# zhanxinrui/HDN

Measured on AMD Instinct MI355X. Metric: frames/sec on 127/255 template/search pairs, higher is better.
Workload: dtype f32; 1 GPU; BASELINE configs[1]: batch=64 synthetic 127/255 pairs per GPU, 256-ch features; HIP kernels only: 1x xcorr 31x31(x)61x61 + 6x xcorr 5x5(x)29x29 + 6x circular xcorr 13x13(x)13x13 + 3x PreShareFeature 127x127 + fused DLT/warp + the 2 L1 scores (one launch); pairs_per_gpu=64, channels=256

## Files before the change

hdn_amd/csrc/share_feature.hip:

```cpp
#include <cstdlib>

#include "hdn_common.h"

#define HDN_ABL_SHARE_FEATURE_0(...) __VA_ARGS__
#define HDN_ABL_SHARE_FEATURE_1(...) __VA_ARGS__
#define HDN_ABL_SHARE_FEATURE_2(...) __VA_ARGS__
#ifdef HDN_ABLATION
#include "ablation/share_feature.inc"
#endif

namespace hdn {

constexpr int SF_ROWS = 4;
constexpr int SF_COLS = 128;

constexpr int SF_W1 = 0, SF_W2 = 36, SF_W3 = 324, SF_ALPHA = 396, SF_BETA = 409;

constexpr int SF_IN_H = SF_ROWS + 6, SF_IN_W = SF_COLS + 6;
constexpr int SF_A_H = SF_ROWS + 4, SF_A_W = SF_COLS + 4;
constexpr int SF_B_H = SF_ROWS + 2, SF_B_W = SF_COLS + 2;
constexpr int SF_IN_N = SF_IN_H * SF_IN_W;
constexpr int SF_A_N = SF_A_H * SF_A_W;
constexpr int SF_B_N = SF_B_H * SF_B_W;
constexpr int SF_LDS_FLOATS = SF_IN_N + 4 * SF_A_N + 8 * SF_B_N;

__global__ __launch_bounds__(HDN_BLOCK) void share_feature_kernel(const float* __restrict__ img,
                                                                  const float* __restrict__ prm,
                                                                  float* __restrict__ out, int H, int W) {
  __shared__ float smem[SF_LDS_FLOATS];
  float* s_in = smem;
  float* s_a = smem + SF_IN_N;
  float* s_b = s_a + 4 * SF_A_N;

  const int tid = threadIdx.x;
  const int c0 = blockIdx.x * SF_COLS;
  const int r0 = blockIdx.y * SF_ROWS;
  const size_t plane = size_t(blockIdx.z) * H * W;
  const float* __restrict__ src = img + plane;

  for (int idx = tid; idx < SF_IN_N; idx += HDN_BLOCK) {
    const int r = idx / SF_IN_W, c = idx - r * SF_IN_W;
    const int gr = r0 - 3 + r, gc = c0 - 3 + c;
    float v = 0.f;
    if (gr >= 0 && gr < H && gc >= 0 && gc < W) v = src[gr * W + gc];
    s_in[idx] = v;
  }
  __syncthreads();

  for (int idx = tid; idx < SF_A_N; idx += HDN_BLOCK) {
    const int r = idx / SF_A_W, c = idx - r * SF_A_W;
    const int gr = r0 - 2 + r, gc = c0 - 2 + c;
    float acc[4] = {0.f, 0.f, 0.f, 0.f};
#pragma unroll
    for (int ky = 0; ky < 3; ++ky)
#pragma unroll
      for (int kx = 0; kx < 3; ++kx) {
        const float v = s_in[(r + ky) * SF_IN_W + c + kx];
#pragma unroll
        for (int co = 0; co < 4; ++co) acc[co] = __builtin_fmaf(v, prm[SF_W1 + (ky * 3 + kx) * 4 + co], acc[co]);
      }
    const bool inside = gr >= 0 && gr < H && gc >= 0 && gc < W;
#pragma unroll
    for (int co = 0; co < 4; ++co) {
      const float y = __builtin_fmaf(acc[co], prm[SF_ALPHA + co], prm[SF_BETA + co]);
      s_a[co * SF_A_N + idx] = inside ? fmaxf(y, 0.f) : 0.f;
    }
  }
  __syncthreads();

  for (int idx = tid; idx < SF_B_N; idx += HDN_BLOCK) {
    const int r = idx / SF_B_W, c = idx - r * SF_B_W;
    const int gr = r0 - 1 + r, gc = c0 - 1 + c;
    float acc[8];
#pragma unroll
    for (int co = 0; co < 8; ++co) acc[co] = 0.f;
#pragma unroll
    for (int ci = 0; ci < 4; ++ci)
#pragma unroll
      for (int ky = 0; ky < 3; ++ky)
#pragma unroll
        for (int kx = 0; kx < 3; ++kx) {
          const float v = s_a[ci * SF_A_N + (r + ky) * SF_A_W + c + kx];
#pragma unroll
          for (int co = 0; co < 8; ++co)
            acc[co] = __builtin_fmaf(v, prm[SF_W2 + (((ci >> 1) * 9 + ky * 3 + kx) * 8 + co) * 2 + (ci & 1)], acc[co]);
        }
    const bool inside = gr >= 0 && gr < H && gc >= 0 && gc < W;
#pragma unroll
    for (int co = 0; co < 8; ++co) {
      const float y = __builtin_fmaf(acc[co], prm[SF_ALPHA + 4 + co], prm[SF_BETA + 4 + co]);
      s_b[co * SF_B_N + idx] = inside ? fmaxf(y, 0.f) : 0.f;
    }
  }
  __syncthreads();

  for (int idx = tid; idx < SF_ROWS * SF_COLS; idx += HDN_BLOCK) {
    const int r = idx / SF_COLS, c = idx - r * SF_COLS;
    const int gr = r0 + r, gc = c0 + c;
    if (gr >= H || gc >= W) continue;
    float acc = 0.f;
#pragma unroll
    for (int ci = 0; ci < 8; ++ci)
#pragma unroll
      for (int ky = 0; ky < 3; ++ky)
#pragma unroll
        for (int kx = 0; kx < 3; ++kx)
          acc = __builtin_fmaf(s_b[ci * SF_B_N + (r + ky) * SF_B_W + c + kx],
                               prm[SF_W3 + ((ci >> 1) * 9 + ky * 3 + kx) * 2 + (ci & 1)], acc);
    const float y = __builtin_fmaf(acc, prm[SF_ALPHA + 12], prm[SF_BETA + 12]);
    out[plane + size_t(gr) * W + gc] = fmaxf(y, 0.f);
  }
}

namespace sfv {
typedef const float __attribute__((address_space(4))) cfloat;
typedef float f16v __attribute__((ext_vector_type(16)));
typedef float f8v __attribute__((ext_vector_type(8)));
typedef float f4v_ __attribute__((ext_vector_type(4)));
typedef const f16v __attribute__((address_space(4), aligned(4))) c16;
typedef const f8v __attribute__((address_space(4), aligned(4))) c8;
typedef const f4v_ __attribute__((address_space(4), aligned(4))) c4;
typedef const float2v __attribute__((address_space(4), aligned(4))) c2;

__device__ __forceinline__ const cfloat* opaque(const float* p) {
  uint64_t a = reinterpret_cast<uint64_t>(p);
  asm volatile("" : "+s"(a));
  return (const cfloat*)a;
}
__device__ __forceinline__ float from_prev_lane(float v) {
  return __builtin_bit_cast(float, __builtin_amdgcn_update_dpp(0, __builtin_bit_cast(int, v), 0x138, 0xf, 0xf, true));
}
__device__ __forceinline__ float from_next_lane(float v) {
  return __builtin_bit_cast(float, __builtin_amdgcn_update_dpp(0, __builtin_bit_cast(int, v), 0x130, 0xf, 0xf, true));
}

#define SFV_FMA_LO(a, v, w) "v_pk_fma_f32 " a ", " v ", " w ", " a " op_sel_hi:[1,0,1]\n\t"
#define SFV_FMA_HI(a, v, w) "v_pk_fma_f32 " a ", " v ", " w ", " a " op_sel:[0,1,0] op_sel_hi:[1,1,1]\n\t"
#define SFV_MUL_LO(a, v, w) "v_pk_mul_f32 " a ", " v ", " w " op_sel_hi:[1,0]\n\t"
#define SFV_MUL_HI(a, v, w) "v_pk_mul_f32 " a ", " v ", " w " op_sel:[0,1] op_sel_hi:[1,1]\n\t"
#define SFV_PAIR(w, k) __builtin_shufflevector(w, w, 2 * (k), 2 * (k) + 1)

template <bool INIT>
__device__ __forceinline__ void tap16(float2v (&acc)[8], float2v ve, float2v vo, const cfloat* wp) {
  const f16v w = *reinterpret_cast<const c16*>(wp);
  if constexpr (INIT) {
    asm(SFV_MUL_LO("%0", "%8", "%10") SFV_MUL_LO("%1", "%8", "%11") SFV_MUL_LO("%2", "%8", "%12") SFV_MUL_LO("%3", "%8", "%13")
        SFV_MUL_LO("%4", "%8", "%14") SFV_MUL_LO("%5", "%8", "%15") SFV_MUL_LO("%6", "%8", "%16") SFV_MUL_LO("%7", "%8", "%17")
        SFV_FMA_HI("%0", "%9", "%10") SFV_FMA_HI("%1", "%9", "%11") SFV_FMA_HI("%2", "%9", "%12") SFV_FMA_HI("%3", "%9", "%13")
        SFV_FMA_HI("%4", "%9", "%14") SFV_FMA_HI("%5", "%9", "%15") SFV_FMA_HI("%6", "%9", "%16") SFV_FMA_HI("%7", "%9", "%17")
        : "=&v"(acc[0]), "=&v"(acc[1]), "=&v"(acc[2]), "=&v"(acc[3]), "=&v"(acc[4]), "=&v"(acc[5]), "=&v"(acc[6]), "=&v"(acc[7])
        : "v"(ve), "v"(vo), "s"(SFV_PAIR(w, 0)), "s"(SFV_PAIR(w, 1)), "s"(SFV_PAIR(w, 2)), "s"(SFV_PAIR(w, 3)), "s"(SFV_PAIR(w, 4)),
          "s"(SFV_PAIR(w, 5)), "s"(SFV_PAIR(w, 6)), "s"(SFV_PAIR(w, 7)));
  } else {
    asm(SFV_FMA_LO("%0", "%8", "%10") SFV_FMA_LO("%1", "%8", "%11") SFV_FMA_LO("%2", "%8", "%12") SFV_FMA_LO("%3", "%8", "%13")
        SFV_FMA_LO("%4", "%8", "%14") SFV_FMA_LO("%5", "%8", "%15") SFV_FMA_LO("%6", "%8", "%16") SFV_FMA_LO("%7", "%8", "%17")
        SFV_FMA_HI("%0", "%9", "%10") SFV_FMA_HI("%1", "%9", "%11") SFV_FMA_HI("%2", "%9", "%12") SFV_FMA_HI("%3", "%9", "%13")
        SFV_FMA_HI("%4", "%9", "%14") SFV_FMA_HI("%5", "%9", "%15") SFV_FMA_HI("%6", "%9", "%16") SFV_FMA_HI("%7", "%9", "%17")
        : "+v"(acc[0]), "+v"(acc[1]), "+v"(acc[2]), "+v"(acc[3]), "+v"(acc[4]), "+v"(acc[5]), "+v"(acc[6]), "+v"(acc[7])
        : "v"(ve), "v"(vo), "s"(SFV_PAIR(w, 0)), "s"(SFV_PAIR(w, 1)), "s"(SFV_PAIR(w, 2)), "s"(SFV_PAIR(w, 3)), "s"(SFV_PAIR(w, 4)),
          "s"(SFV_PAIR(w, 5)), "s"(SFV_PAIR(w, 6)), "s"(SFV_PAIR(w, 7)));
  }
}

template <bool INIT>
__device__ __forceinline__ void scatter18(float2v& o0, float2v& o1, float2v& o2, float2v& o3, float2v& o4, float2v& o5, float2v& o6,
                                          float2v& o7, float2v& o8, float2v be, float2v bo, const cfloat* wp) {
  const f16v w = *reinterpret_cast<const c16*>(wp);
  const float2v w8 = *reinterpret_cast<const c2*>(wp + 16);
  if constexpr (INIT) {
    asm(SFV_MUL_LO("%0", "%9", "%11") SFV_MUL_LO("%1", "%9", "%12") SFV_MUL_LO("%2", "%9", "%13") SFV_FMA_LO("%3", "%9", "%14")
        SFV_FMA_LO("%4", "%9", "%15") SFV_FMA_LO("%5", "%9", "%16") SFV_FMA_LO("%6", "%9", "%17") SFV_FMA_LO("%7", "%9", "%18")
        SFV_FMA_LO("%8", "%9", "%19")
        SFV_FMA_HI("%0", "%10", "%11") SFV_FMA_HI("%1", "%10", "%12") SFV_FMA_HI("%2", "%10", "%13") SFV_FMA_HI("%3", "%10", "%14")
        SFV_FMA_HI("%4", "%10", "%15") SFV_FMA_HI("%5", "%10", "%16") SFV_FMA_HI("%6", "%10", "%17") SFV_FMA_HI("%7", "%10", "%18")
        SFV_FMA_HI("%8", "%10", "%19")
        : "=&v"(o0), "=&v"(o1), "=&v"(o2), "+v"(o3), "+v"(o4), "+v"(o5), "+v"(o6), "+v"(o7), "+v"(o8)
        : "v"(be), "v"(bo), "s"(SFV_PAIR(w, 0)), "s"(SFV_PAIR(w, 1)), "s"(SFV_PAIR(w, 2)), "s"(SFV_PAIR(w, 3)), "s"(SFV_PAIR(w, 4)),
          "s"(SFV_PAIR(w, 5)), "s"(SFV_PAIR(w, 6)), "s"(SFV_PAIR(w, 7)), "s"(w8));
  } else {
    asm(SFV_FMA_LO("%0", "%9", "%11") SFV_FMA_LO("%1", "%9", "%12") SFV_FMA_LO("%2", "%9", "%13") SFV_FMA_LO("%3", "%9", "%14")
        SFV_FMA_LO("%4", "%9", "%15") SFV_FMA_LO("%5", "%9", "%16") SFV_FMA_LO("%6", "%9", "%17") SFV_FMA_LO("%7", "%9", "%18")
        SFV_FMA_LO("%8", "%9", "%19")
        SFV_FMA_HI("%0", "%10", "%11") SFV_FMA_HI("%1", "%10", "%12") SFV_FMA_HI("%2", "%10", "%13") SFV_FMA_HI("%3", "%10", "%14")
        SFV_FMA_HI("%4", "%10", "%15") SFV_FMA_HI("%5", "%10", "%16") SFV_FMA_HI("%6", "%10", "%17") SFV_FMA_HI("%7", "%10", "%18")
        SFV_FMA_HI("%8", "%10", "%19")
        : "+v"(o0), "+v"(o1), "+v"(o2), "+v"(o3), "+v"(o4), "+v"(o5), "+v"(o6), "+v"(o7), "+v"(o8)
        : "v"(be), "v"(bo), "s"(SFV_PAIR(w, 0)), "s"(SFV_PAIR(w, 1)), "s"(SFV_PAIR(w, 2)), "s"(SFV_PAIR(w, 3)), "s"(SFV_PAIR(w, 4)),
          "s"(SFV_PAIR(w, 5)), "s"(SFV_PAIR(w, 6)), "s"(SFV_PAIR(w, 7)), "s"(w8));
  }
}

template <bool INIT>
__device__ __forceinline__ void l1row(float2v (&acc)[4], float2v i0, float2v i1, float2v i2, const cfloat* wp) {
  const f8v w = *reinterpret_cast<const c8*>(wp);
  const f4v_ u = *reinterpret_cast<const c4*>(wp + 8);
  if constexpr (INIT) {
    asm(SFV_MUL_LO("%0", "%4", "%7") SFV_MUL_HI("%1", "%4", "%7") SFV_MUL_LO("%2", "%4", "%8") SFV_MUL_HI("%3", "%4", "%8")
        SFV_FMA_LO("%0", "%5", "%9") SFV_FMA_HI("%1", "%5", "%9") SFV_FMA_LO("%2", "%5", "%10") SFV_FMA_HI("%3", "%5", "%10")
        SFV_FMA_LO("%0", "%6", "%11") SFV_FMA_HI("%1", "%6", "%11") SFV_FMA_LO("%2", "%6", "%12") SFV_FMA_HI("%3", "%6", "%12")
        : "=&v"(acc[0]), "=&v"(acc[1]), "=&v"(acc[2]), "=&v"(acc[3])
        : "v"(i0), "v"(i1), "v"(i2), "s"(SFV_PAIR(w, 0)), "s"(SFV_PAIR(w, 1)), "s"(SFV_PAIR(w, 2)), "s"(SFV_PAIR(w, 3)),
          "s"(SFV_PAIR(u, 0)), "s"(SFV_PAIR(u, 1)));
  } else {
    asm(SFV_FMA_LO("%0", "%4", "%7") SFV_FMA_HI("%1", "%4", "%7") SFV_FMA_LO("%2", "%4", "%8") SFV_FMA_HI("%3", "%4", "%8")
        SFV_FMA_LO("%0", "%5", "%9") SFV_FMA_HI("%1", "%5", "%9") SFV_FMA_LO("%2", "%5", "%10") SFV_FMA_HI("%3", "%5", "%10")
        SFV_FMA_LO("%0", "%6", "%11") SFV_FMA_HI("%1", "%6", "%11") SFV_FMA_LO("%2", "%6", "%12") SFV_FMA_HI("%3", "%6", "%12")
        : "+v"(acc[0]), "+v"(acc[1]), "+v"(acc[2]), "+v"(acc[3])
        : "v"(i0), "v"(i1), "v"(i2), "s"(SFV_PAIR(w, 0)), "s"(SFV_PAIR(w, 1)), "s"(SFV_PAIR(w, 2)), "s"(SFV_PAIR(w, 3)),
          "s"(SFV_PAIR(u, 0)), "s"(SFV_PAIR(u, 1)));
  }
}

__device__ __forceinline__ float2v bn_relu(float2v acc, float2v ab) {
  asm("v_pk_fma_f32 %0, %0, %1, %1 op_sel:[0,0,1] op_sel_hi:[1,0,1]" : "+v"(acc) : "v"(ab));
  float lo = acc.x, hi = acc.y;
  asm("v_max_f32 %0, 0, %0" : "+v"(lo));
  asm("v_max_f32 %0, 0, %0" : "+v"(hi));
  return float2v{lo, hi};
}

struct State {
  float2v in[3][3];
  float2v a[3][4][3];
  float2v o[3][3];
  float2v ab[13];
};

struct Ctx {
  const float* __restrict__ src;
  float* __restrict__ dst;
  const float* __restrict__ prm;
  int H, W, ra, rb;
  int col0, col1;
  bool m0, m1;
};

__device__ __forceinline__ float2v load_row(const Ctx& c, int i) {
  const bool row_ok = i >= 0 && i < c.H;
  const float* __restrict__ p = c.src + (row_ok ? i : 0) * c.W;
  const float x0 = p[c.col0], x1 = p[c.col1];
  return float2v{row_ok && c.m0 ? x0 : 0.f, row_ok && c.m1 ? x1 : 0.f};
}

template <int PH, bool FULL>
__device__ __forceinline__ void step(State& st, const Ctx& c, int i, float2v xin) {
  constexpr int S0 = PH, S1 = (PH + 2) % 3, S2 = (PH + 1) % 3;
  const cfloat* prm = opaque(c.prm);
  st.in[S0][1] = xin;
  st.in[S0][0] = float2v{from_prev_lane(xin.y), xin.x};
  st.in[S0][2] = float2v{xin.y, from_next_lane(xin.x)};

  const int sg = i - 1;
  if (FULL || sg >= c.ra - 2) {
    if (FULL || (sg >= 0 && sg < c.H)) {
      const cfloat* w1 = prm + SF_W1;
      float2v acc[4];
      l1row<true>(acc, st.in[S2][0], st.in[S2][1], st.in[S2][2], w1);
      l1row<false>(acc, st.in[S1][0], st.in[S1][1], st.in[S1][2], w1 + 12);
      l1row<false>(acc, st.in[S0][0], st.in[S0][1], st.in[S0][2], w1 + 24);
#pragma unroll
      for (int co = 0; co < 4; ++co) {
        float2v y = bn_relu(acc[co], st.ab[co]);
        y.x = c.m0 ? y.x : 0.f;
        y.y = c.m1 ? y.y : 0.f;
        st.a[S1][co][1] = y;
        st.a[S1][co][0] = float2v{from_prev_lane(y.y), y.x};
        st.a[S1][co][2] = float2v{y.y, from_next_lane(y.x)};
      }
    } else {
#pragma unroll
      for (int co = 0; co < 4; ++co)
#pragma unroll
        for (int kx = 0; kx < 3; ++kx) st.a[S1][co][kx] = float2v{0.f, 0.f};
    }
  }

  const int rho = i - 2;
  if (FULL || (rho >= c.ra - 1 && rho >= 0 && rho < c.H)) {
    float2v acc[8];
#pragma unroll
    for (int ky = 0; ky < 3; ++ky) {
      constexpr int rs_[3] = {S0, S2, S1};
      const int rs = rs_[ky];
#pragma unroll
      for (int cp = 0; cp < 2; ++cp) {
        const cfloat* w = prm + SF_W2 + (cp * 3 + ky) * 48;
#pragma unroll
        for (int kx = 0; kx < 3; ++kx) {
          if (ky == 0 && cp == 0 && kx == 0) tap16<true>(acc, st.a[rs][2 * cp][kx], st.a[rs][2 * cp + 1][kx], w + kx * 16);
          else tap16<false>(acc, st.a[rs][2 * cp][kx], st.a[rs][2 * cp + 1][kx], w + kx * 16);
        }
      }
    }
#pragma unroll
    for (int co = 0; co < 8; ++co) acc[co] = bn_relu(acc[co], st.ab[4 + co]);
    const cfloat* w3 = prm + SF_W3;
    scatter18<true>(st.o[S1][0], st.o[S1][1], st.o[S1][2], st.o[S2][0], st.o[S2][1], st.o[S2][2], st.o[S0][0], st.o[S0][1], st.o[S0][2],
                    acc[0], acc[1], w3);
#pragma unroll
    for (int cq = 1; cq < 4; ++cq)
      scatter18<false>(st.o[S1][0], st.o[S1][1], st.o[S1][2], st.o[S2][0], st.o[S2][1], st.o[S2][2], st.o[S0][0], st.o[S0][1], st.o[S0][2],
                       acc[2 * cq], acc[2 * cq + 1], w3 + cq * 18);
  } else {
#pragma unroll
    for (int kx = 0; kx < 3; ++kx) st.o[S1][kx] = float2v{0.f, 0.f};
  }

  const int orow = i - 3;
  if (FULL || (orow >= c.ra && orow < c.rb)) {
    asm volatile("s_nop 1");
    const float2v A = st.o[S0][0], B = st.o[S0][1];
    float2v C = st.o[S0][2];
    C.x = c.m0 ? C.x : 0.f;
    C.y = c.m1 ? C.y : 0.f;
    const float2v r = bn_relu(float2v{from_prev_lane(A.y) + B.x + C.y, A.x + B.y + from_next_lane(C.x)}, st.ab[12]);
    float* __restrict__ q = c.dst + size_t(orow) * c.W;
    if (c.m0) q[c.col0] = r.x;
    if (c.m1) q[c.col1] = r.y;
  }
}

template <bool FULL>
__device__ __forceinline__ bool round3(State& st, const Ctx& c, int i, int last, float2v& x) {
  float2v xn = load_row(c, i + 1);
  step<0, FULL>(st, c, i, x);
  if (!FULL && i + 1 > last) return true;
  x = load_row(c, i + 2);
  step<1, FULL>(st, c, i + 1, xn);
  if (!FULL && i + 2 > last) return true;
  xn = load_row(c, i + 3);
  step<2, FULL>(st, c, i + 2, x);
  x = xn;
  return !FULL && i + 3 > last;
}
}

__global__ __launch_bounds__(HDN_BLOCK) void share_feature_rows_kernel(const float* __restrict__ img, const float* __restrict__ prm,
                                                                       float* __restrict__ out, int H, int W, int rows_per_strip,
                                                                       int strips_per_img, int total_strips) {
  using namespace sfv;
  HDN_ABL_SHARE_FEATURE_0()
  const int lane = threadIdx.x & 63;
  const int strip = __builtin_amdgcn_readfirstlane(blockIdx.x * (HDN_BLOCK / 64) + (threadIdx.x >> 6));
  if (strip >= total_strips) return;
  const int bimg = strip / strips_per_img, k = strip - bimg * strips_per_img;
  Ctx c;
  c.src = img + size_t(bimg) * H * W;
  c.dst = out + size_t(bimg) * H * W;
  c.prm = prm;
  c.H = H;
  c.W = W;
  c.ra = k * rows_per_strip;
  c.rb = min(c.ra + rows_per_strip, H);
  c.m0 = 2 * lane < W;
  c.m1 = 2 * lane + 1 < W;
  c.col0 = c.m0 ? 2 * lane : 0;
  c.col1 = c.m1 ? 2 * lane + 1 : 0;
  State st;
#pragma unroll
  for (int s = 0; s < 3; ++s)
#pragma unroll
    for (int kx = 0; kx < 3; ++kx) {
      st.in[s][kx] = float2v{0.f, 0.f};
      st.o[s][kx] = float2v{0.f, 0.f};
#pragma unroll
      for (int ch = 0; ch < 4; ++ch) st.a[s][ch][kx] = float2v{0.f, 0.f};
    }
#pragma unroll
  for (int ch = 0; ch < 13; ++ch) {
    st.ab[ch] = float2v{prm[SF_ALPHA + ch], prm[SF_BETA + ch]};
    asm volatile("" : "+v"(st.ab[ch]));
  }
  if (rows_per_strip == 1) {
    float2v xr[7];
#pragma unroll
    for (int q = 0; q < 7; ++q) xr[q] = load_row(c, c.ra - 3 + q);
    HDN_ABL_SHARE_FEATURE_1()
    HDN_ABL_SHARE_FEATURE_2()
    step<0, false>(st, c, c.ra - 3, xr[0]);
    step<1, false>(st, c, c.ra - 2, xr[1]);
    step<2, false>(st, c, c.ra - 1, xr[2]);
    step<0, false>(st, c, c.ra, xr[3]);
    step<1, false>(st, c, c.ra + 1, xr[4]);
    step<2, false>(st, c, c.ra + 2, xr[5]);
    step<0, false>(st, c, c.ra + 3, xr[6]);
    return;
  }
  const int last = c.rb + 2;
  const int full_lo = c.ra + 3, full_hi = min(c.rb + 2, H - 1);
  int i = c.ra - 3;
  float2v x = load_row(c, i);
#pragma unroll 1
  for (;;) {
    if (round3<false>(st, c, i, last, x)) break;
    i += 3;
    if (i >= full_lo) {
#pragma unroll 1
      while (i + 2 <= full_hi) {
        round3<true>(st, c, i, last, x);
        i += 3;
      }
    }
  }
}

static int launch_sf_rows(const float* img, const float* folded, float* out, int B, int H, int W, hipStream_t stream) {
  static const int forced = [] { const char* e = getenv("HDN_SF_STRIP"); return e ? atoi(e) : 0; }();
  int n = (long long)B * H <= 1024 ? 1 : 2;
  while (n < H && (long long)B * cdiv(H, n) > 3072) n *= 2;
  if (forced > 0) n = forced;
  const int strips = cdiv(H, n);
  const long long total = (long long)strips * B;
  if (total > 0x7fffffffLL) return HDN_E_LIMIT;
  const int wpb = HDN_BLOCK / 64;
  hipLaunchKernelGGL(share_feature_rows_kernel, dim3((unsigned)((total + wpb - 1) / wpb)), dim3(HDN_BLOCK), 0, stream, img, folded, out,
                     H, W, n, strips, (int)total);
  return launch_status();
}

}

extern "C" int hdn_share_feature_f32(const float* img, const float* folded, float* out, int B, int H, int W,
                                     void* stream) {
  if (!img || !folded || !out) return HDN_E_NULL;
  if (B <= 0 || H <= 0 || W <= 0) return HDN_E_SHAPE;
  if (B > 65535 || (long long)H * W > 0x7fffffffLL / 4) return HDN_E_LIMIT;
  if (out == img) return HDN_E_ALIAS;
  if (W <= 128) {
    return hdn::launch_sf_rows(img, folded, out, B, H, W, static_cast<hipStream_t>(stream));
  }
  dim3 grid(hdn::cdiv(W, hdn::SF_COLS), hdn::cdiv(H, hdn::SF_ROWS), B);
  if (grid.y > 65535) return HDN_E_LIMIT;
  hipLaunchKernelGGL(hdn::share_feature_kernel, grid, dim3(HDN_BLOCK), 0, static_cast<hipStream_t>(stream), img, folded,
                     out, H, W);
  return hdn::launch_status();
}
```

Measured before the change: 234,400 frames/s.

## Add streamed row kernel that software-pipelines weight and input row loads

Adds a second row-strip kernel variant whose condition-free steps prefetch the next conv tap's scalar weights while the current tap's packed FMAs run, with volatile loads and asm dependency fences to enforce the ordering. Input rows are also loaded three rows ahead as raw values. The host picks the streamed kernel when the strip count exceeds 1024, which covers B=64, H=127 with 2-row strips. The aim is to hide scalar-load latency on the weight reads, at the cost of more live registers and possibly lower occupancy.

Result: no change. 235,000 frames/s, median of 2 (+0.2%).

```diff
diff --git a/hdn_amd/csrc/share_feature.hip b/hdn_amd/csrc/share_feature.hip
--- a/hdn_amd/csrc/share_feature.hip
+++ b/hdn_amd/csrc/share_feature.hip
@@ -141,8 +141,7 @@
 #define SFV_PAIR(w, k) __builtin_shufflevector(w, w, 2 * (k), 2 * (k) + 1)
 
 template <bool INIT>
-__device__ __forceinline__ void tap16(float2v (&acc)[8], float2v ve, float2v vo, const cfloat* wp) {
-  const f16v w = *reinterpret_cast<const c16*>(wp);
+__device__ __forceinline__ void tap16w(float2v (&acc)[8], float2v ve, float2v vo, const f16v w) {
   if constexpr (INIT) {
     asm(SFV_MUL_LO("%0", "%8", "%10") SFV_MUL_LO("%1", "%8", "%11") SFV_MUL_LO("%2", "%8", "%12") SFV_MUL_LO("%3", "%8", "%13")
         SFV_MUL_LO("%4", "%8", "%14") SFV_MUL_LO("%5", "%8", "%15") SFV_MUL_LO("%6", "%8", "%16") SFV_MUL_LO("%7", "%8", "%17")
@@ -163,10 +162,13 @@
 }
 
 template <bool INIT>
-__device__ __forceinline__ void scatter18(float2v& o0, float2v& o1, float2v& o2, float2v& o3, float2v& o4, float2v& o5, float2v& o6,
-                                          float2v& o7, float2v& o8, float2v be, float2v bo, const cfloat* wp) {
-  const f16v w = *reinterpret_cast<const c16*>(wp);
-  const float2v w8 = *reinterpret_cast<const c2*>(wp + 16);
+__device__ __forceinline__ void tap16(float2v (&acc)[8], float2v ve, float2v vo, const cfloat* wp) {
+  tap16w<INIT>(acc, ve, vo, *reinterpret_cast<const c16*>(wp));
+}
+
+template <bool INIT>
+__device__ __forceinline__ void scatter18w(float2v& o0, float2v& o1, float2v& o2, float2v& o3, float2v& o4, float2v& o5, float2v& o6,
+                                           float2v& o7, float2v& o8, float2v be, float2v bo, const f16v w, const float2v w8) {
   if constexpr (INIT) {
     asm(SFV_MUL_LO("%0", "%9", "%11") SFV_MUL_LO("%1", "%9", "%12") SFV_MUL_LO("%2", "%9", "%13") SFV_FMA_LO("%3", "%9", "%14")
         SFV_FMA_LO("%4", "%9", "%15") SFV_FMA_LO("%5", "%9", "%16") SFV_FMA_LO("%6", "%9", "%17") SFV_FMA_LO("%7", "%9", "%18")
@@ -191,9 +193,13 @@
 }
 
 template <bool INIT>
-__device__ __forceinline__ void l1row(float2v (&acc)[4], float2v i0, float2v i1, float2v i2, const cfloat* wp) {
-  const f8v w = *reinterpret_cast<const c8*>(wp);
-  const f4v_ u = *reinterpret_cast<const c4*>(wp + 8);
+__device__ __forceinline__ void scatter18(float2v& o0, float2v& o1, float2v& o2, float2v& o3, float2v& o4, float2v& o5, float2v& o6,
+                                          float2v& o7, float2v& o8, float2v be, float2v bo, const cfloat* wp) {
+  scatter18w<INIT>(o0, o1, o2, o3, o4, o5, o6, o7, o8, be, bo, *reinterpret_cast<const c16*>(wp), *reinterpret_cast<const c2*>(wp + 16));
+}
+
+template <bool INIT>
+__device__ __forceinline__ void l1roww(float2v (&acc)[4], float2v i0, float2v i1, float2v i2, const f8v w, const f4v_ u) {
   if constexpr (INIT) {
     asm(SFV_MUL_LO("%0", "%4", "%7") SFV_MUL_HI("%1", "%4", "%7") SFV_MUL_LO("%2", "%4", "%8") SFV_MUL_HI("%3", "%4", "%8")
         SFV_FMA_LO("%0", "%5", "%9") SFV_FMA_HI("%1", "%5", "%9") SFV_FMA_LO("%2", "%5", "%10") SFV_FMA_HI("%3", "%5", "%10")
@@ -211,12 +217,42 @@
   }
 }
 
+template <bool INIT>
+__device__ __forceinline__ void l1row(float2v (&acc)[4], float2v i0, float2v i1, float2v i2, const cfloat* wp) {
+  l1roww<INIT>(acc, i0, i1, i2, *reinterpret_cast<const c8*>(wp), *reinterpret_cast<const c4*>(wp + 8));
+}
+
 __device__ __forceinline__ float2v bn_relu(float2v acc, float2v ab) {
   asm("v_pk_fma_f32 %0, %0, %1, %1 op_sel:[0,0,1] op_sel_hi:[1,0,1]" : "+v"(acc) : "v"(ab));
   float lo = acc.x, hi = acc.y;
   asm("v_max_f32 %0, 0, %0" : "+v"(lo));
   asm("v_max_f32 %0, 0, %0" : "+v"(hi));
   return float2v{lo, hi};
+}
+
+struct L1W {
+  f8v w[3];
+  f4v_ u[3];
+};
+__device__ __forceinline__ L1W load_l1w(const cfloat* prm) {
+  L1W l;
+#pragma unroll
+  for (int ky = 0; ky < 3; ++ky) {
+    l.w[ky] = *reinterpret_cast<const volatile c8*>(prm + SF_W1 + 12 * ky);
+    l.u[ky] = *reinterpret_cast<const volatile c4*>(prm + SF_W1 + 12 * ky + 8);
+  }
+  return l;
+}
+template <class T>
+__device__ __forceinline__ const cfloat* arrived(const cfloat* p, const T& chunk, float2v& done) {
+  uint64_t a = reinterpret_cast<uint64_t>(p);
+  asm volatile("" : "+s"(a), "+v"(done) : "s"(chunk));
+  return (const cfloat*)a;
+}
+__device__ __forceinline__ void asked(float2v& v) { asm volatile("" : "+v"(v)); }
+__device__ __forceinline__ f16v load_tap(const cfloat* prm, int t) {
+  const int kx = t % 3, cp = (t / 3) & 1, ky = t / 6;
+  return *reinterpret_cast<const volatile c16*>(prm + SF_W2 + (cp * 3 + ky) * 48 + kx * 16);
 }
 
 struct State {
@@ -242,22 +278,38 @@
   return float2v{row_ok && c.m0 ? x0 : 0.f, row_ok && c.m1 ? x1 : 0.f};
 }
 
-template <int PH, bool FULL>
+template <int PH, bool FULL, bool PIPE = false>
 __device__ __forceinline__ void step(State& st, const Ctx& c, int i, float2v xin) {
+  static_assert(FULL || !PIPE, "only a condition-free step streams its weights");
   constexpr int S0 = PH, S1 = (PH + 2) % 3, S2 = (PH + 1) % 3;
   const cfloat* prm = opaque(c.prm);
+  L1W l1;
+  if constexpr (PIPE) {
+    l1 = load_l1w(prm);
+  }
   st.in[S0][1] = xin;
   st.in[S0][0] = float2v{from_prev_lane(xin.y), xin.x};
   st.in[S0][2] = float2v{xin.y, from_next_lane(xin.x)};
 
+  f16v t2;
   const int sg = i - 1;
   if (FULL || sg >= c.ra - 2) {
     if (FULL || (sg >= 0 && sg < c.H)) {
       const cfloat* w1 = prm + SF_W1;
       float2v acc[4];
-      l1row<true>(acc, st.in[S2][0], st.in[S2][1], st.in[S2][2], w1);
-      l1row<false>(acc, st.in[S1][0], st.in[S1][1], st.in[S1][2], w1 + 12);
-      l1row<false>(acc, st.in[S0][0], st.in[S0][1], st.in[S0][2], w1 + 24);
+      if constexpr (PIPE) {
+        prm = arrived(prm, l1.w[0], st.in[S0][2]);
+        t2 = load_tap(prm, 0);
+        float2v first = st.in[S2][0];
+        asked(first);
+        l1roww<true>(acc, first, st.in[S2][1], st.in[S2][2], l1.w[0], l1.u[0]);
+        l1roww<false>(acc, st.in[S1][0], st.in[S1][1], st.in[S1][2], l1.w[1], l1.u[1]);
+        l1roww<false>(acc, st.in[S0][0], st.in[S0][1], st.in[S0][2], l1.w[2], l1.u[2]);
+      } else {
+        l1row<true>(acc, st.in[S2][0], st.in[S2][1], st.in[S2][2], w1);
+        l1row<false>(acc, st.in[S1][0], st.in[S1][1], st.in[S1][2], w1 + 12);
+        l1row<false>(acc, st.in[S0][0], st.in[S0][1], st.in[S0][2], w1 + 24);
+      }
 #pragma unroll
       for (int co = 0; co < 4; ++co) {
         float2v y = bn_relu(acc[co], st.ab[co]);
@@ -278,29 +330,78 @@
   const int rho = i - 2;
   if (FULL || (rho >= c.ra - 1 && rho >= 0 && rho < c.H)) {
     float2v acc[8];
-#pragma unroll
-    for (int ky = 0; ky < 3; ++ky) {
-      constexpr int rs_[3] = {S0, S2, S1};
-      const int rs = rs_[ky];
-#pragma unroll
-      for (int cp = 0; cp < 2; ++cp) {
-        const cfloat* w = prm + SF_W2 + (cp * 3 + ky) * 48;
-#pragma unroll
-        for (int kx = 0; kx < 3; ++kx) {
-          if (ky == 0 && cp == 0 && kx == 0) tap16<true>(acc, st.a[rs][2 * cp][kx], st.a[rs][2 * cp + 1][kx], w + kx * 16);
-          else tap16<false>(acc, st.a[rs][2 * cp][kx], st.a[rs][2 * cp + 1][kx], w + kx * 16);
-        }
-      }
-    }
-#pragma unroll
-    for (int co = 0; co < 8; ++co) acc[co] = bn_relu(acc[co], st.ab[4 + co]);
-    const cfloat* w3 = prm + SF_W3;
-    scatter18<true>(st.o[S1][0], st.o[S1][1], st.o[S1][2], st.o[S2][0], st.o[S2][1], st.o[S2][2], st.o[S0][0], st.o[S0][1], st.o[S0][2],
-                    acc[0], acc[1], w3);
-#pragma unroll
-    for (int cq = 1; cq < 4; ++cq)
-      scatter18<false>(st.o[S1][0], st.o[S1][1], st.o[S1][2], st.o[S2][0], st.o[S2][1], st.o[S2][2], st.o[S0][0], st.o[S0][1], st.o[S0][2],
-                       acc[2 * cq], acc[2 * cq + 1], w3 + cq * 18);
+    constexpr int rs_[3] = {S0, S2, S1};
+    if constexpr (PIPE) {
+      f16v d;
+      float2v d8;
+#pragma unroll
+      for (int t = 0; t < 18; ++t) {
+        prm = arrived(prm, t2, t == 0 ? st.a[S1][3][2] : acc[0]);
+        f16v n;
+        if (t < 17) {
+          n = load_tap(prm, t + 1);
+        } else {
+          d = *reinterpret_cast<const volatile c16*>(prm + SF_W3);
+          d8 = *reinterpret_cast<const volatile c2*>(prm + SF_W3 + 16);
+        }
+        const int kx = t % 3, cp = (t / 3) & 1, rs = rs_[t / 6];
+        if (t == 0) {
+          float2v first = st.a[rs][0][0];
+          asked(first);
+          tap16w<true>(acc, first, st.a[rs][1][0], t2);
+        } else {
+          asked(acc[0]);
+          tap16w<false>(acc, st.a[rs][2 * cp][kx], st.a[rs][2 * cp + 1][kx], t2);
+        }
+        if (t < 17) t2 = n;
+      }
+#pragma unroll
+      for (int co = 0; co < 8; ++co) acc[co] = bn_relu(acc[co], st.ab[4 + co]);
+#pragma unroll
+      for (int cq = 0; cq < 4; ++cq) {
+        prm = arrived(prm, d, cq == 0 ? acc[7] : st.o[S2][0]);
+        f16v nd;
+        float2v nd8;
+        if (cq < 3) {
+          nd = *reinterpret_cast<const volatile c16*>(prm + SF_W3 + (cq + 1) * 18);
+          nd8 = *reinterpret_cast<const volatile c2*>(prm + SF_W3 + (cq + 1) * 18 + 16);
+          asked(st.o[S2][0]);
+        }
+        if (cq == 0)
+          scatter18w<true>(st.o[S1][0], st.o[S1][1], st.o[S1][2], st.o[S2][0], st.o[S2][1], st.o[S2][2], st.o[S0][0], st.o[S0][1], st.o[S0][2],
+                           acc[0], acc[1], d, d8);
+        else
+          scatter18w<false>(st.o[S1][0], st.o[S1][1], st.o[S1][2], st.o[S2][0], st.o[S2][1], st.o[S2][2], st.o[S0][0], st.o[S0][1], st.o[S0][2],
+                            acc[2 * cq], acc[2 * cq + 1], d, d8);
+        if (cq < 3) {
+          d = nd;
+          d8 = nd8;
+        }
+      }
+    } else {
+#pragma unroll
+      for (int ky = 0; ky < 3; ++ky) {
+        const int rs = rs_[ky];
+#pragma unroll
+        for (int cp = 0; cp < 2; ++cp) {
+          const cfloat* w = prm + SF_W2 + (cp * 3 + ky) * 48;
+#pragma unroll
+          for (int kx = 0; kx < 3; ++kx) {
+            if (ky == 0 && cp == 0 && kx == 0) tap16<true>(acc, st.a[rs][2 * cp][kx], st.a[rs][2 * cp + 1][kx], w + kx * 16);
+            else tap16<false>(acc, st.a[rs][2 * cp][kx], st.a[rs][2 * cp + 1][kx], w + kx * 16);
+          }
+        }
+      }
+#pragma unroll
+      for (int co = 0; co < 8; ++co) acc[co] = bn_relu(acc[co], st.ab[4 + co]);
+      const cfloat* w3 = prm + SF_W3;
+      scatter18<true>(st.o[S1][0], st.o[S1][1], st.o[S1][2], st.o[S2][0], st.o[S2][1], st.o[S2][2], st.o[S0][0], st.o[S0][1], st.o[S0][2],
+                      acc[0], acc[1], w3);
+#pragma unroll
+      for (int cq = 1; cq < 4; ++cq)
+        scatter18<false>(st.o[S1][0], st.o[S1][1], st.o[S1][2], st.o[S2][0], st.o[S2][1], st.o[S2][2], st.o[S0][0], st.o[S0][1], st.o[S0][2],
+                         acc[2 * cq], acc[2 * cq + 1], w3 + cq * 18);
+    }
   } else {
 #pragma unroll
     for (int kx = 0; kx < 3; ++kx) st.o[S1][kx] = float2v{0.f, 0.f};
@@ -333,12 +434,39 @@
   x = xn;
   return !FULL && i + 3 > last;
 }
-}
-
-__global__ __launch_bounds__(HDN_BLOCK) void share_feature_rows_kernel(const float* __restrict__ img, const float* __restrict__ prm,
-                                                                       float* __restrict__ out, int H, int W, int rows_per_strip,
-                                                                       int strips_per_img, int total_strips) {
-  using namespace sfv;
+
+struct RawRow {
+  float x0, x1;
+};
+__device__ __forceinline__ RawRow load_raw(const Ctx& c, int i) {
+  const float* __restrict__ p = c.src + (i >= 0 && i < c.H ? i : 0) * c.W;
+  return RawRow{p[c.col0], p[c.col1]};
+}
+__device__ __forceinline__ float2v use_row(const Ctx& c, int i, RawRow r) {
+  asm volatile("" : "+v"(r.x0), "+v"(r.x1));
+  const bool row_ok = i >= 0 && i < c.H;
+  return float2v{row_ok && c.m0 ? r.x0 : 0.f, row_ok && c.m1 ? r.x1 : 0.f};
+}
+
+template <bool FULL>
+__device__ __forceinline__ bool round3_stream(State& st, const Ctx& c, int i, int last, RawRow (&q)[3]) {
+  const RawRow n0 = load_raw(c, i + 3);
+  step<0, FULL, FULL>(st, c, i, use_row(c, i, q[0]));
+  if (!FULL && i + 1 > last) return true;
+  const RawRow n1 = load_raw(c, i + 4);
+  step<1, FULL, FULL>(st, c, i + 1, use_row(c, i + 1, q[1]));
+  if (!FULL && i + 2 > last) return true;
+  const RawRow n2 = load_raw(c, i + 5);
+  step<2, FULL, FULL>(st, c, i + 2, use_row(c, i + 2, q[2]));
+  q[0] = n0;
+  q[1] = n1;
+  q[2] = n2;
+  return !FULL && i + 3 > last;
+}
+
+template <bool STREAM>
+__device__ __forceinline__ void rows_strip(const float* __restrict__ img, const float* __restrict__ prm, float* __restrict__ out, int H, int W,
+                                           int rows_per_strip, int strips_per_img, int total_strips) {
   HDN_ABL_SHARE_FEATURE_0()
   const int lane = threadIdx.x & 63;
   const int strip = __builtin_amdgcn_readfirstlane(blockIdx.x * (HDN_BLOCK / 64) + (threadIdx.x >> 6));
@@ -371,7 +499,7 @@
     st.ab[ch] = float2v{prm[SF_ALPHA + ch], prm[SF_BETA + ch]};
     asm volatile("" : "+v"(st.ab[ch]));
   }
-  if (rows_per_strip == 1) {
+  if (!STREAM && rows_per_strip == 1) {
     float2v xr[7];
 #pragma unroll
     for (int q = 0; q < 7; ++q) xr[q] = load_row(c, c.ra - 3 + q);
@@ -389,32 +517,65 @@
   const int last = c.rb + 2;
   const int full_lo = c.ra + 3, full_hi = min(c.rb + 2, H - 1);
   int i = c.ra - 3;
-  float2v x = load_row(c, i);
+  if constexpr (STREAM) {
+    RawRow q[3] = {load_raw(c, i), load_raw(c, i + 1), load_raw(c, i + 2)};
 #pragma unroll 1
-  for (;;) {
-    if (round3<false>(st, c, i, last, x)) break;
-    i += 3;
-    if (i >= full_lo) {
+    for (;;) {
+      if (round3_stream<false>(st, c, i, last, q)) break;
+      i += 3;
+      if (i >= full_lo) {
 #pragma unroll 1
-      while (i + 2 <= full_hi) {
-        round3<true>(st, c, i, last, x);
-        i += 3;
-      }
-    }
-  }
+        while (i + 2 <= full_hi) {
+          round3_stream<true>(st, c, i, last, q);
+          i += 3;
+        }
+      }
+    }
+  } else {
+    float2v x = load_row(c, i);
+#pragma unroll 1
+    for (;;) {
+      if (round3<false>(st, c, i, last, x)) break;
+      i += 3;
+      if (i >= full_lo) {
+#pragma unroll 1
+        while (i + 2 <= full_hi) {
+          round3<true>(st, c, i, last, x);
+          i += 3;
+        }
+      }
+    }
+  }
+}
+}
+
+__global__ __launch_bounds__(HDN_BLOCK) void share_feature_rows_kernel(const float* __restrict__ img, const float* __restrict__ prm,
+                                                                       float* __restrict__ out, int H, int W, int rows_per_strip,
+                                                                       int strips_per_img, int total_strips) {
+  sfv::rows_strip<false>(img, prm, out, H, W, rows_per_strip, strips_per_img, total_strips);
+}
+
+__global__ __launch_bounds__(HDN_BLOCK) void share_feature_rows_stream_kernel(const float* __restrict__ img, const float* __restrict__ prm,
+                                                                            float* __restrict__ out, int H, int W, int rows_per_strip,
+                                                                            int strips_per_img, int total_strips) {
+  sfv::rows_strip<true>(img, prm, out, H, W, rows_per_strip, strips_per_img, total_strips);
 }
 
 static int launch_sf_rows(const float* img, const float* folded, float* out, int B, int H, int W, hipStream_t stream) {
   static const int forced = [] { const char* e = getenv("HDN_SF_STRIP"); return e ? atoi(e) : 0; }();
   int n = (long long)B * H <= 1024 ? 1 : 2;
   while (n < H && (long long)B * cdiv(H, n) > 3072) n *= 2;
-  if (forced > 0) n = forced;
+  bool streamed = (long long)B * cdiv(H, n) > 1024;
+  if (forced > 0) {
+    n = forced;
+    streamed = n >= 16;
+  }
   const int strips = cdiv(H, n);
   const long long total = (long long)strips * B;
   if (total > 0x7fffffffLL) return HDN_E_LIMIT;
   const int wpb = HDN_BLOCK / 64;
-  hipLaunchKernelGGL(share_feature_rows_kernel, dim3((unsigned)((total + wpb - 1) / wpb)), dim3(HDN_BLOCK), 0, stream, img, folded, out,
-                     H, W, n, strips, (int)total);
+  hipLaunchKernelGGL(streamed ? share_feature_rows_stream_kernel : share_feature_rows_kernel, dim3((unsigned)((total + wpb - 1) / wpb)),
+                     dim3(HDN_BLOCK), 0, stream, img, folded, out, H, W, n, strips, (int)total);
   return launch_status();
 }
 
```
